# zaphB/freecad.optics_design_workbench

Measured on AMD Instinct MI355X. Metric: Monte-Carlo rays/sec (whole node), lensesAndMirrors.FCStd, higher is better.
Workload: dtype f64; 1 GPU; benchmark/lensesAndMirrors.FCStd, 1e+08 Monte-Carlo rays per step per GPU (BASELINE configs[2]), Gaussian point source sigma=1e-2, Philox4x32-10 seed 0x0D15EA5E; record_hit_rows=True, histogram=1024x1024 u64, parallelism=ray-index sharding x1, one RCCL reduce

## Files before the change

### freecad/optics_design_workbench_amd/csrc/odw_capi.hip

```cpp
#include <hip/hip_runtime.h>
#include <hipcub/hipcub.hpp>

#include <algorithm>
#include <array>
#include <cmath>
#include <cstdio>
#include <cstdlib>
#include <cstring>
#include <condition_variable>
#include <functional>
#include <mutex>
#include <new>
#include <thread>
#include <string>
#include <utility>
#include <vector>

#include "odw_kernels.hip"
#include "odw_grid.hip"
#include "odw_mesh.hip"

using namespace odw;

namespace {
// ... 2150 lines not shown
  }
  return ODW_OK;
}

namespace {
void batch_unselect(odw_ctx* ctx) {
  if (ctx->batch_selected < 0 && !ctx->archive_selected) return;
  ctx->archive_selected = false;
  ctx->hits = ctx->own_hits;
  ctx->hit_count = ctx->own_hit_count;
  ctx->hit_capacity = ctx->own_capacity;
  ctx->hit_slots = ctx->own_slots;
  ctx->hit_ray_begin = ctx->own_ray_begin;
  ctx->hit_ray_end = ctx->own_ray_end;
  ctx->own_hits = DevBuf();
  ctx->own_hit_count = DevBuf();
  ctx->batch_selected = -1;
  ctx->ph_valid = false;
}

bool same_structure(const odw_ctx& a, const odw_ctx& b, std::string& why) {
  if (a.P.scene.n_prims != b.P.scene.n_prims || a.P.scene.n_groups != b.P.scene.n_groups) { why = "primitive or group count"; return false; }
  for (size_t i = 0; i < a.h_prim_i32.size(); ++i) {
    const int32_t mask = (i % 4 == 2) ? ~(int32_t)ODW_FLAG_ISOLATED : ~0;
    if ((a.h_prim_i32[i] & mask) != (b.h_prim_i32[i] & mask)) { why = "primitive kinds, groups, flags or trimming lists"; return false; }
  }
  if (a.h_cond != b.h_cond) { why = "trimming conditions"; return false; }
  if (a.h_group_i32 != b.h_group_i32) { why = "optical types / recording switches / grating kinds"; return false; }
  if (a.h_seq != b.h_seq || a.P.scene.seq_enabled != b.P.scene.seq_enabled || a.P.scene.seq_len != b.P.scene.seq_len ||
      a.P.scene.ignore_mask != b.P.scene.ignore_mask) { why = "tracing sequence / ignored groups"; return false; }
  if (a.lean != b.lean) { why = "gratings or absorbing media in some scenes only"; return false; }
  return true;
}
}

int odw_upload_scene_batch(odw_ctx* ctx, const odw_scene_desc* scenes, int32_t n_scenes) {
  if (!ctx || !scenes || n_scenes < 1) return fail(ctx, ODW_ERR_INVALID, "odw_upload_scene_batch: bad argument");
  if (!ctx->have_limits) return fail(ctx, ODW_ERR_NO_SCENE, "odw_upload_scene_batch before odw_set_limits (the boxes carry the tolerance)");
  HIPCHK(ctx, hipSetDevice(ctx->device));
  ctx->batch_n = 0;
  ctx->batch_traced = 0;
  ctx->batch_rows_ok = false;
  ctx->phb_valid = ctx->phb_projected = false;
  int rc = odw_upload_scene(ctx, &scenes[0]);
  if (rc) return rc;
  if ((rc = build_bvh(ctx))) return rc;
  if (ctx->P.scene.n_nodes || ctx->P.grid.nx > 0)
    return fail(ctx, ODW_ERR_UNSUPPORTED, "odw_upload_scene_batch: batches are traced by the flat kernels (analytic scenes of up to 64 primitives)");
  const bool compiled = ctx->compile_mode != ODW_COMPILE_OFF && spec_ineligible(ctx).empty();
  const std::string text0 = compiled ? spec_text(ctx) : std::string();
  const size_t n = (size_t)ctx->P.scene.n_prims;
  const size_t o_hdr = 16 * n, o_gf = o_hdr + 8 * n, o_gd = o_gf + ODW_MAX_GROUPS * 4, stride = o_gd + ODW_MAX_GROUPS * 3;
  std::vector<double> blocks(stride * (size_t)n_scenes, 0.0);
  for (int k = 0; k < n_scenes; ++k) {
    odw_ctx tmp;
    std::memset(&tmp.P, 0, sizeof tmp.P);
    if ((rc = scene_host_tables(&tmp, &scenes[k]))) { ctx->err = tmp.err; g_error = tmp.err; return rc; }
    std::string why;
    if (!same_structure(*ctx, tmp, why))
      return fail(ctx, ODW_ERR_UNSUPPORTED, "odw_upload_scene_batch: scene " + std::to_string(k) + " differs from scene 0 in structure (" + why + ")");
    tmp.P.lim = ctx->P.lim;
    tmp.have_limits = true;
    std::vector<Box> boxes;
    std::vector<char> dead;
    compute_boxes(&tmp, boxes, dead);
    if (compiled && spec_text(&tmp) != text0)
      return fail(ctx, ODW_ERR_UNSUPPORTED, "odw_upload_scene_batch: scene " + std::to_string(k) + " differs from scene 0 in the structure a "
                                            "compiled kernel is built from (which frame entries are 0 / +1 / -1, shared boxes)");
    double* b = blocks.data() + stride * (size_t)k;
    std::memcpy(b, tmp.h_prim_f64.data(), 16 * n * sizeof(double));
    std::memcpy(b + o_hdr, tmp.h_prim_hdr.data(), 8 * n * sizeof(double));
    for (size_t p = 0; p < n; ++p) {
      int32_t w[4];
      std::memcpy(w, b + o_hdr + 8 * p + 6, sizeof w);
      w[2] &= ~ODW_FLAG_ISOLATED;
      std::memcpy(b + o_hdr + 8 * p + 6, w, sizeof w);
    }
    std::memcpy(b + o_gf, tmp.h_group_f64.data(), ODW_MAX_GROUPS * 4 * sizeof(double));
    std::memcpy(b + o_gd, tmp.h_group_gdir.data(), ODW_MAX_GROUPS * 3 * sizeof(double));
  }
  if ((rc = upload(ctx, ctx->batch_values, blocks.data(), blocks.size() * sizeof(double)))) return rc;
  std::vector<int32_t> pi = ctx->h_prim_i32;
  for (size_t p = 0; p < n; ++p) pi[4 * p + 2] &= ~ODW_FLAG_ISOLATED;
  if (n && (rc = upload(ctx, ctx->prim_i32, pi.data(), pi.size() * sizeof(int32_t)))) return rc;
  if ((rc = upload_done(ctx))) return rc;
  ctx->h_prim_i32 = pi;
  ctx->batch_n = n_scenes;
  ctx->batch_prims = n;
  ctx->batch_stride = stride;
  ctx->batch_spec_text = text0;
  return ODW_OK;
}

namespace {
uint64_t batch_slots(odw_ctx* ctx, uint64_t rows_per_scene) {
  uint64_t slots = rows_per_scene;
  if (rows_per_scene >= kHitBlockMinRows)
    slots += hit_block_room(rows_per_scene, std::min<uint64_t>((uint64_t)ctx->n_cu * 8 * 4, std::max<uint64_t>(64, rows_per_scene / 256)), kHitBlock);
  return slots;
}
}

int odw_batch_reserve(odw_ctx* ctx, int32_t n_scenes, uint64_t rays_per_scene, uint64_t rows_per_scene) {
  if (!ctx || n_scenes < 1 || rays_per_scene == 0) return fail(ctx, ODW_ERR_INVALID, "odw_batch_reserve: bad argument");
  HIPCHK(ctx, hipSetDevice(ctx->device));
  const uint64_t S = (uint64_t)n_scenes, slots = batch_slots(ctx, rows_per_scene);
  if (slots > 0x7FFFFFFFull) return fail(ctx, ODW_ERR_CAPACITY, "odw_batch_reserve: more than 2^31 rows per scene");
  HIPCHK(ctx, hipStreamSynchronize(ctx->stream));
  int rc = ODW_OK;
  if (rows_per_scene) {
    rc = ensure(ctx, ctx->batch_hits, S * slots * sizeof(odw_hit));
    if (!rc) rc = ensure(ctx, ctx->batch_hit_count, S * 4 * sizeof(uint64_t));
  }
  if (!rc) rc = phb_reserve(ctx, (int)S, rays_per_scene, slots);
  if (!rc && rows_per_scene && rays_per_scene <= (1ull << 28))
    rc = ensure(ctx, ctx->phb_pts, S * slots * 3 * sizeof(double));
  if (!rc && S >= 3) rc = ensure(ctx, ctx->batch_rays_buf, (size_t)((rays_per_scene + 31) / 32 * 32 * 6 + 4) * sizeof(double));
  return rc;
}

int odw_trace_batch(odw_ctx* ctx, uint64_t first_ray, uint64_t rays_per_scene, uint64_t seed, uint32_t flags,
                    uint64_t rows_per_scene) {
  if (!ctx) return fail(ctx, ODW_ERR_INVALID, "odw_trace_batch: null ctx");
  if (ctx->batch_n < 1)
    return fail(ctx, ODW_ERR_NO_SCENE, "odw_trace_batch before odw_upload_scene_batch (odw_upload_scene and a new dist_tol discard an uploaded batch)");
  if (ctx->bvh_dirty || (size_t)ctx->P.scene.n_prims != ctx->batch_prims)
    return fail(ctx, ODW_ERR_NO_SCENE, "odw_trace_batch: the scene changed after odw_upload_scene_batch");
  if (ctx->emitter_active) return fail(ctx, ODW_ERR_UNSUPPORTED, "odw_trace_batch: point sources only");
  if (rays_per_scene == 0) return ODW_OK;
  HIPCHK(ctx, hipSetDevice(ctx->device));
  batch_unselect(ctx);
  ctx->batch_rows_ok = false;
  const uint64_t S = (uint64_t)ctx->batch_n;
  if (flags & ODW_TRACE_RECORD_HITS) {
    if (rows_per_scene == 0) return fail(ctx, ODW_ERR_CAPACITY, "odw_trace_batch: ODW_TRACE_RECORD_HITS with rows_per_scene = 0");
    const uint64_t slots = batch_slots(ctx, rows_per_scene);
// ... 515 lines not shown
```

### freecad/optics_design_workbench_amd/csrc/odw_device.h

```cpp
#pragma once
#ifndef __HIPCC_RTC__
#include <hip/hip_runtime.h>
#include <stdint.h>
#else
typedef signed char int8_t;
typedef unsigned char uint8_t;
typedef signed int int32_t;
typedef unsigned int uint32_t;
typedef signed long int64_t;
typedef unsigned long uint64_t;
typedef unsigned long uintptr_t;
#endif

#ifdef __HIPCC_RTC__
#include "odw_trace.h"
#else
#include "../../../include/odw_trace.h"
#endif

#ifndef INFINITY
#define INFINITY (__builtin_inff())
#endif

namespace odw {

#define ODW_TAG_UNUSED 0xFFFFFFFFFFFFFFFFull
#define ODW_CNT_LDS 8
#define ODW_SOLID_SHIFT 16
#define ODW_FLAG_ISOLATED 0x4

__host__ __device__ __forceinline__ constexpr int cond_operand(int cw) { return cw & 0x3fffffff; }
__host__ __device__ __forceinline__ constexpr bool cond_opens(int cw) { return (cw & 0x40000000) != 0; }

struct d3 {
  double x, y, z;
};
__device__ __forceinline__ d3 mk(double x, double y, double z) { return d3{x, y, z}; }
__device__ __forceinline__ d3 operator+(d3 a, d3 b) { return mk(a.x + b.x, a.y + b.y, a.z + b.z); }
__device__ __forceinline__ d3 operator-(d3 a, d3 b) { return mk(a.x - b.x, a.y - b.y, a.z - b.z); }
__device__ __forceinline__ d3 operator*(d3 a, double s) { return mk(a.x * s, a.y * s, a.z * s); }
__device__ __forceinline__ double dot(d3 a, d3 b) { return a.x * b.x + a.y * b.y + a.z * b.z; }
__device__ __forceinline__ d3 cross(d3 a, d3 b) {
  return mk(a.y * b.z - a.z * b.y, a.z * b.x - a.x * b.z, a.x * b.y - a.y * b.x);
}
__device__ __forceinline__ double comp(d3 a, int i) { return i == 0 ? a.x : (i == 1 ? a.y : a.z); }

struct DeviceScene {
  const double* prim_f64;
  const double* prim_hdr;
  const int32_t* prim_i32;
  const int32_t* cond_i32;
  const double* group_f64;
  const int32_t* group_i32;
  const double* group_gdir;
  const uint64_t* seq_mask;
  const float* bvh_nodes;
  const int32_t* bvh_prims;
  const float* bvh_leaf;
  const uint32_t* bvh_wide;
  double wide_lo[3], wide_hi[3];
  const double* tri_nrm;
  int32_t n_prims, n_groups, n_nodes;
  int32_t seq_enabled, seq_len;
  uint64_t ignore_mask, all_mask;
};

struct DeviceGrid {
  const double* bounds;
  const uint32_t* cells;
  const void* items;
  int32_t nx, ny, nz, n_items;
  int32_t spheres;
  int32_t in_lds;
  uint32_t lds_bytes;
};

struct DeviceSource {
  double m[12];
  double focal_length, wavelength, power;
  const double* phi_tab;
  const double* t_tab;
  const int32_t* t_guide;
  const int32_t* phi_guide;
  int32_t n_phi_knots, n_t_knots, n_t_rows, n_guide, n_phi_guide;
  int32_t finite_focal;
};

struct DeviceSurfaceSampler {
  const double* phi_tab;
  const double* t_tab;
  const int32_t* t_guide;
  int32_t n_phi_knots, n_t_knots, n_t_rows, n_guide;
  int32_t axis, n_family;
  double lo, inv_step;
  double mu;
  int32_t next;
  int32_t n_atoms;
  const double* atom_mass;
// ... 79 lines not shown
```

### freecad/optics_design_workbench_amd/csrc/odw_grid.hip

```cpp
#include "odw_device.h"

namespace odw {

#ifndef ODW_GRID_STEP_MIN
#define ODW_GRID_STEP_MIN 24
#endif
#ifndef ODW_GRID_REFILL_MIN
#define ODW_GRID_REFILL_MIN 1
#endif
#define ODW_GRID_THREADS 1024
#define ODW_GRID_WAVES (ODW_GRID_THREADS / 64)
#define ODW_GRID_WAVE_WORDS 32
#define ODW_GRID_RING 64
#define ODW_GRID_RING_DOUBLES (ODW_GRID_RING * 7)

#ifdef ODW_GRID_STATS
#define ODW_GSTAT(k, mask_)                                                                           \
  do {                                                                                                \
    const unsigned long long m_ = (mask_);                                                            \
    if (m_ && (int)__lane_id() == __ffsll(m_) - 1) { wave_cnt[8 + 2 * (k)] += 1u; wave_cnt[9 + 2 * (k)] += (uint32_t)__popcll(m_); } \
  } while (0)
#define ODW_GTIME(k) do { const uint64_t t_ = __builtin_readcyclecounter(); phase_t[(k)] += t_ - t_mark; t_mark = t_; } while (0)
#else
#define ODW_GSTAT(k, mask_) do {} while (0)
#define ODW_GTIME(k) do {} while (0)
#endif

__device__ __forceinline__ double fmin_raw(double a, double b) {
  double r;
  asm("v_min_f64 %0, %1, %2" : "=v"(r) : "v"(a), "v"(b));
  return r;
}

__device__ __forceinline__ int grid_slab(const double* b, int n, double v) {
  int lo = 0, hi = n;
  while (hi - lo > 1) {
    const int mid = (lo + hi) >> 1;
    if (v >= b[mid]) lo = mid; else hi = mid;
  }
  return lo;
}

#define ODW_GCOUNT(k) atomicAdd(&wave_cnt[(k)], 1u)

template <bool SPHERES, bool IN_LDS>
__global__ __launch_bounds__(ODW_GRID_THREADS) void odw_grid_kernel(const TraceParams P) {
  extern __shared__ double grid_lds[];
  const DeviceScene& sc = P.scene;
  const DeviceLimits& lim = P.lim;
  const DeviceGrid& GD = P.grid;
  const int nx = GD.nx, ny = GD.ny, nz = GD.nz;
  const int nb = nx + ny + nz + 3;
  const int ncell = nx * ny * nz;
  uint32_t* lds32 = reinterpret_cast<uint32_t*>(grid_lds);
  const int word_off = 2 * nb;
  const int ring_off = (word_off + ODW_GRID_WAVES * ODW_GRID_WAVE_WORDS + 1) / 2;
  const int cell_off = 2 * (ring_off + ODW_GRID_WAVES * ODW_GRID_RING_DOUBLES);
  const int item_off = ((cell_off + (IN_LDS ? ncell : 0) + 3) & ~3) / 2;
  for (int k = threadIdx.x; k < nb; k += ODW_GRID_THREADS) grid_lds[k] = GD.bounds[k];
  for (int k = threadIdx.x; k < ODW_GRID_WAVES * ODW_GRID_WAVE_WORDS; k += ODW_GRID_THREADS)
    lds32[word_off + k] = (k % ODW_GRID_WAVE_WORDS) == 30 ? P.out.hit_block : 0u;
  if (IN_LDS) {
    for (int k = threadIdx.x; k < ncell; k += ODW_GRID_THREADS) lds32[cell_off + k] = GD.cells[k];
    const int n_words = SPHERES ? GD.n_items * 6 : (GD.n_items + 1) / 2;
    const double* src = reinterpret_cast<const double*>(GD.items);
    for (int k = threadIdx.x; k < n_words; k += ODW_GRID_THREADS) grid_lds[item_off + k] = src[k];
  }
  __syncthreads();
  const double* bx = grid_lds;
  const int by_off = nx + 1, bz_off = nx + ny + 2;
  const int wave = threadIdx.x >> 6;
  uint32_t* wave_cnt = lds32 + word_off + wave * ODW_GRID_WAVE_WORDS;
  volatile uint32_t* hit_state = wave_cnt + 28;
  double* ring = grid_lds + ring_off + wave * ODW_GRID_RING_DOUBLES;

  SceneView sv;
  sv.prim_f64 = as_const(sc.prim_f64);
  sv.prim_hdr = as_const(sc.prim_hdr);
  sv.prim_i32 = as_const(sc.prim_i32);
  sv.cond_i32 = as_const(sc.cond_i32);
  __shared__ double group_f64[64 * 4];
  __shared__ int32_t group_i32[64 * 4];
  __shared__ double group_gdir[64 * 3];
  {
    cf64 gf = as_const(sc.group_f64);
// ... 400 lines not shown
```

### freecad/optics_design_workbench_amd/csrc/odw_kernels.hip

```cpp
#include "odw_device.h"

namespace odw {

#define ODW_CONST __attribute__((address_space(4)))
typedef const double ODW_CONST* cf64;
typedef const int32_t ODW_CONST* ci32;
typedef const uint64_t ODW_CONST* cu64;
template <class T>
__device__ __forceinline__ const T ODW_CONST* as_const(const T* p) {
  return (const T ODW_CONST*)(uintptr_t)p;
}
template <class T>
__device__ __forceinline__ const T* opaque(const T* p) {
  asm volatile("" : "+s"(p));
  return p;
}
typedef const DeviceSource ODW_CONST* csource;
typedef const DeviceDetector ODW_CONST* cdetector;

__device__ __forceinline__ double frcp(double x) {
  double r = __builtin_amdgcn_rcp(x);
  r = fma(fma(-x, r, 1.0), r, r);
  r = fma(fma(-x, r, 1.0), r, r);
  return r;
// ... 318 lines not shown
    }
    if (!held) return;
  }
  if (cand_any) { q.any.t = t; q.any.prim = p; q.any.face = face; }
  if (cand_oth) { q.oth.t = t; q.oth.prim = p; q.oth.face = face; }
}

template <bool PARAB, class SPEC, int C, int END>
__device__ __forceinline__ bool trim_all(const SceneView& sv, const Query& q, d3 gp) {
  if constexpr (C >= END) {
    return true;
  } else {
    constexpr int cw = SPEC::cond(C);
    constexpr int qp = cond_operand(cw);
    cf64 pf = sv.prim_f64 + (size_t)qp * 16;
    const double sd = prim_sdist<PARAB>(SPEC::type(qp), pf + 12, xf_point_nz<SPEC::xf(qp)>(pf, gp));
    if (cw < 0) { if (sd > q.tol) return false; }
    else { if (sd < -q.tol) return false; }
    return trim_all<PARAB, SPEC, C + 1, END>(sv, q, gp);
  }
}
template <class SPEC>
__host__ __device__ constexpr int clause_end(int c, int end) {
  int e = c + 1;
  while (e < end && !cond_opens(SPEC::cond(e))) ++e;
  return e;
}
template <bool PARAB, class SPEC, int C, int END>
__device__ __forceinline__ bool trim_ok(const SceneView& sv, const Query& q, d3 gp) {
  constexpr int E = clause_end<SPEC>(C, END);
  if constexpr (E >= END) {
    return trim_all<PARAB, SPEC, C, END>(sv, q, gp);
  } else {
    if (trim_all<PARAB, SPEC, C, E>(sv, q, gp)) return true;
    return trim_ok<PARAB, SPEC, E, END>(sv, q, gp);
  }
}
template <bool PARAB, class SPEC, int PI>
__device__ __forceinline__ void consider_spec(const SceneView& sv, Query& q, double t, int face) {
  if (!(t > q.tol && t < q.tmax)) return;
  const int key = (PI << 8) | face;
#define ODW_BETTER(B) ((bool)((int)(t < (B).t) | ((int)(t == (B).t) & (int)(key < (B).face))))
  const bool cand_any = ODW_BETTER(q.any);
  bool cand_oth = false;
  if (q.in_medium) cand_oth = (SPEC::group(PI) != q.medium) && (q.medium >= 0) && ODW_BETTER(q.oth);
#undef ODW_BETTER
  if (!cand_any && !cand_oth) return;
  if constexpr (SPEC::cond_cnt(PI) > 0) {
    if (!trim_ok<PARAB, SPEC, SPEC::cond_off(PI), SPEC::cond_off(PI) + SPEC::cond_cnt(PI)>(sv, q, q.start + q.dn * t)) return;
#if ODW_DOUBLE == 5
    if (!trim_ok<PARAB, SPEC, SPEC::cond_off(PI), SPEC::cond_off(PI) + SPEC::cond_cnt(PI)>(sv, q, q.start + q.dn * opq(t))) return;
#endif
  }
  if (cand_any) { q.any.t = t; q.any.face = key; q.cut = fmin(q.tmax, t + 2.0 * q.tol); }
  if (cand_oth) { q.oth.t = t; q.oth.face = key; }
}

struct Cands {
  double t0, t1, t2, t3;
  int f0, f1, f2, f3;
};
__device__ __forceinline__ void cand_push(Cands& c, int& n, double t, int f) {
  if (n == 0) { c.t0 = t; c.f0 = f; }
  else if (n == 1) { c.t1 = t; c.f1 = f; }
  else if (n == 2) { c.t2 = t; c.f2 = f; }
  else { c.t3 = t; c.f3 = f; }
  ++n;
}
__device__ __forceinline__ void cand_min2(Cands& c, double t, int f) {
  const bool lt0 = t < c.t0 || (t == c.t0 && f < c.f0);
  const bool lt1 = t < c.t1 || (t == c.t1 && f < c.f1);
  c.t1 = lt0 ? c.t0 : (lt1 ? t : c.t1);
  c.f1 = lt0 ? c.f0 : (lt1 ? f : c.f1);
  c.t0 = lt0 ? t : c.t0;
  c.f0 = lt0 ? f : c.f0;
}

#ifndef ODW_TORUS_PLAIN
#define ODW_TORUS_PLAIN 96
#endif
template <bool PARAB = true, class SPEC = NoSpec, int PI = 0>
__device__ __forceinline__ void intersect_prim(const SceneView& sv, Query& q, int p, int type, int group,
                                               int flags, int cond_word) {
  cf64 pf = sv.prim_f64 + (size_t)p * 16;
  const int cond_off = cond_word & 0xffffff, cond_cnt = (cond_word >> 24) & 0xff;
  const int fmask = (flags >> ODW_FACEMASK_SHIFT) & 0xff;
  cf64 par = pf + 12;
  const double tol = q.tol;
  Cands c;
  c.t0 = c.t1 = c.t2 = c.t3 = INFINITY;
  c.f0 = c.f1 = c.f2 = c.f3 = 0;
  if (type == ODW_PRIM_SPHERE) {
    if (fmask & 1) {
      const d3 oc = q.start - mk(par[1], par[2], par[3]);
      double t0, t1;
      if (quad_roots_unit(dot(oc, q.dn), dot(oc, oc) - par[0] * par[0], t0, t1) == 2) {
        c.t0 = t0;
        c.t1 = t1;
      }
#if ODW_DOUBLE == 2
      {
        const d3 oc2 = mk(opq(oc.x), oc.y, oc.z);
        double u0 = INFINITY, u1 = INFINITY;
        if (quad_roots_unit(dot(oc2, q.dn), dot(oc2, oc2) - par[0] * par[0], u0, u1) == 2) { c.t0 = u0 == c.t0 ? c.t0 : u0; c.t1 = u1 == c.t1 ? c.t1 : u1; }
      }
#endif
    }
  } else {
  d3 o, d;
  if constexpr (SPEC::enabled) {
    o = xf_point_nz<SPEC::xf(PI)>(pf, q.start);
    d = xf_vec_nz<SPEC::xf(PI)>(pf, q.dn);
  } else {
    o = xf_point(pf, q.start);
    d = xf_vec(pf, q.dn);
  }
  if (type == ODW_PRIM_BOX) {
    const double ix = frcp(d.x), iy = frcp(d.y), iz = frcp(d.z);
    const double ax = -o.x * ix, ay = -o.y * iy, az = -o.z * iz;
    const double bx = fma(par[0], ix, ax), by = fma(par[1], iy, ay), bz = fma(par[2], iz, az);
    const bool px = d.x > 0, py = d.y > 0, pz = d.z > 0;
    const double nx_ = fmin(ax, bx), ny_ = fmin(ay, by), nz_ = fmin(az, bz);
    const double fx_ = fmax(ax, bx), fy_ = fmax(ay, by), fz_ = fmax(az, bz);
    if (cond_cnt) {
#define ODW_BOX_FACE2(T, FACE, P1, D1, S1, P2, D2, S2, TA, FA, TB, FB)                          \
      {                                                                                         \
        const double t_ = (T);                                                                  \
        const double u_ = fma(t_, D1, P1), v_ = fma(t_, D2, P2);                                \
        const bool ok_ = ((fmask >> (FACE)) & 1) && t_ > tol && u_ >= -tol && u_ <= (S1) + tol && \
                         v_ >= -tol && v_ <= (S2) + tol;                                        \
        const bool a_ = ok_ && t_ < TA;                                                         \
        const bool b_ = ok_ && !a_ && t_ < TB;                                                  \
        TB = a_ ? TA : (b_ ? t_ : TB);                                                          \
        FB = a_ ? FA : (b_ ? (FACE) : FB);                                                      \
        TA = a_ ? t_ : TA;                                                                      \
        FA = a_ ? (FACE) : FA;                                                                  \
      }
      ODW_BOX_FACE2(nx_, px ? 0 : 1, o.y, d.y, par[1], o.z, d.z, par[2], c.t0, c.f0, c.t2, c.f2);
      ODW_BOX_FACE2(ny_, py ? 2 : 3, o.z, d.z, par[2], o.x, d.x, par[0], c.t0, c.f0, c.t2, c.f2);
      ODW_BOX_FACE2(nz_, pz ? 4 : 5, o.x, d.x, par[0], o.y, d.y, par[1], c.t0, c.f0, c.t2, c.f2);
      ODW_BOX_FACE2(fx_, px ? 1 : 0, o.y, d.y, par[1], o.z, d.z, par[2], c.t1, c.f1, c.t3, c.f3);
      ODW_BOX_FACE2(fy_, py ? 3 : 2, o.z, d.z, par[2], o.x, d.x, par[0], c.t1, c.f1, c.t3, c.f3);
      ODW_BOX_FACE2(fz_, pz ? 5 : 4, o.x, d.x, par[0], o.y, d.y, par[1], c.t1, c.f1, c.t3, c.f3);
#undef ODW_BOX_FACE2
    } else {
    double bt = INFINITY;
    int bf = 0;
#define ODW_BOX_OK(A, B, C, D, E, F) (bool)((int)(A) & (int)(B) & (int)(C) & (int)(D) & (int)(E) & (int)(F))
#define ODW_BOX_FACE(T, FACE, P1, D1, S1, P2, D2, S2)                                         \
    {                                                                                         \
      const double t_ = (T);                                                                  \
      const double u_ = fma(t_, D1, P1), v_ = fma(t_, D2, P2);                                \
      const bool ok_ = ODW_BOX_OK(((fmask >> (FACE)) & 1) != 0, t_ > tol, u_ >= -tol, u_ <= (S1) + tol, \
                                  v_ >= -tol, v_ <= (S2) + tol);                              \
      if (ok_ && (t_ < bt || (t_ == bt && (FACE) < bf))) { bt = t_; bf = (FACE); }            \
    }
    ODW_BOX_FACE(nx_, px ? 0 : 1, o.y, d.y, par[1], o.z, d.z, par[2]);
    ODW_BOX_FACE(ny_, py ? 2 : 3, o.z, d.z, par[2], o.x, d.x, par[0]);
    ODW_BOX_FACE(nz_, pz ? 4 : 5, o.x, d.x, par[0], o.y, d.y, par[1]);
    c.t0 = bt;
    c.f0 = bf;
    const double t_in = fmax(fmax(nx_, ny_), nz_);
    const double t_out = fmin(fmin(fx_, fy_), fz_);
    if (!(bt < INFINITY) || !(t_in < t_out)) {
      bt = INFINITY;
      bf = 0;
      ODW_BOX_FACE(fx_, px ? 1 : 0, o.y, d.y, par[1], o.z, d.z, par[2]);
      ODW_BOX_FACE(fy_, py ? 3 : 2, o.z, d.z, par[2], o.x, d.x, par[0]);
      ODW_BOX_FACE(fz_, pz ? 5 : 4, o.x, d.x, par[0], o.y, d.y, par[1]);
      c.t1 = bt;
      c.f1 = bf;
    }
#undef ODW_BOX_FACE
#undef ODW_BOX_OK
    }
  } else if (type == ODW_PRIM_CYLINDER || type == ODW_PRIM_CONE || (PARAB && type == ODW_PRIM_PARABOLOID)) {
    const bool parab = PARAB && type == ODW_PRIM_PARABOLOID;
    const double R1 = parab ? 0.0 : par[0];
    const double R2 = (type == ODW_PRIM_CYLINDER) ? par[0] : (parab ? par[2] : par[1]);
    const double H = (type == ODW_PRIM_CONE) ? par[2] : par[1];
    const double k = (type == ODW_PRIM_CONE) ? (R2 - R1) / H : 0.0;
    const double f2 = parab ? 2.0 * par[0] : 0.0;
    constexpr bool side_skip = SPEC::enabled || !PARAB;
    bool side = (fmask & 1) != 0;
    double invz = 0.0;
    if ((fmask & 6) || (side_skip && type == ODW_PRIM_CYLINDER && side)) invz = frcp(d.z);
    if (side_skip && type == ODW_PRIM_CYLINDER && side) {
      const double tl = (-tol - o.z) * invz, th = (H + tol - o.z) * invz;
      const double xl = fma(tl, d.x, o.x), yl = fma(tl, d.y, o.y), xh = fma(th, d.x, o.x), yh = fma(th, d.y, o.y);
      const double lim = R1 * R1 * (1.0 - 1e-9);
      side = !(fma(xl, xl, yl * yl) < lim && fma(xh, xh, yh * yh) < lim);
    }
    if (side) {
      const double rz = R1 + k * o.z;
      double t0 = INFINITY, t1 = INFINITY;
      const int nr = quad_roots(d.x * d.x + d.y * d.y - k * k * d.z * d.z,
                                o.x * d.x + o.y * d.y - k * rz * d.z - f2 * d.z,
                                o.x * o.x + o.y * o.y - rz * rz - 2.0 * f2 * o.z, t0, t1);
      const double z0 = o.z + t0 * d.z, z1 = o.z + t1 * d.z;
      c.t0 = (bool)((int)(nr >= 1) & (int)(z0 >= -tol) & (int)(z0 <= H + tol) & (int)((R1 + k * z0) >= -tol)) ? t0 : c.t0;
      c.t1 = (bool)((int)(nr == 2) & (int)(z1 >= -tol) & (int)(z1 <= H + tol) & (int)((R1 + k * z1) >= -tol)) ? t1 : c.t1;
    }
    if (fmask & 6) {
      const double ta = (0.0 - o.z) * invz, tb = (H - o.z) * invz;
      const double xa = o.x + ta * d.x, ya = o.y + ta * d.y;
      const double xb = o.x + tb * d.x, yb = o.y + tb * d.y;
      { const bool w_ = (bool)((int)((fmask & 2) != 0) & (int)(R1 > 0) & (int)(xa * xa + ya * ya <= (R1 + tol) * (R1 + tol))); c.t2 = w_ ? ta : c.t2; c.f2 = w_ ? 1 : c.f2; }
      { const bool w_ = (bool)((int)((fmask & 4) != 0) & (int)(R2 > 0) & (int)(xb * xb + yb * yb <= (R2 + tol) * (R2 + tol))); c.t3 = w_ ? tb : c.t3; c.f3 = w_ ? 2 : c.f3; }
    }
  } else {
    if (!(fmask & 1)) return;
    const double R1 = par[0], R2 = par[1];
    const double t0 = -dot(o, d);
    const d3 cc = o + d * t0;
    const double bound = (R1 + R2) * 1.0000001 + 1e-9;
    const double h2 = bound * bound - dot(cc, cc);
// ... 138 lines not shown
}

__device__ __forceinline__ d3 tri_normal(cf64 pf, const double* __restrict__ vn, d3 gp) {
  const d3 ng = mk(pf[9], pf[10], pf[11]);
  if (!vn) return ng;
  const d3 e1 = mk(pf[3], pf[4], pf[5]), e2 = mk(pf[6], pf[7], pf[8]);
  const d3 tv = gp - mk(pf[0], pf[1], pf[2]);
  const d3 nn = cross(e1, e2);
  const double inv = frcp(dot(nn, nn));
  const double u = dot(cross(tv, e2), nn) * inv, v = dot(cross(e1, tv), nn) * inv;
  const double w = 1.0 - u - v;
  const d3 n = mk(w * vn[0] + u * vn[3] + v * vn[6], w * vn[1] + u * vn[4] + v * vn[7],
                  w * vn[2] + u * vn[5] + v * vn[8]);
  const double l2 = dot(n, n);
  return l2 > 0 ? n * frsqrt(l2) : ng;
}

template <bool PARAB = true>
__device__ __forceinline__ d3 face_normal(int type, cf64 par, int face, d3 lp) {
  if (type == ODW_PRIM_BOX) {
    const double s = (face & 1) ? 1.0 : -1.0;
    const int a = face >> 1;
    return mk(a == 0 ? s : 0.0, a == 1 ? s : 0.0, a == 2 ? s : 0.0);
  }
  if (type == ODW_PRIM_SPHERE) return lp * frsqrt(dot(lp, lp));
  if (type == ODW_PRIM_CYLINDER || type == ODW_PRIM_CONE || (PARAB && type == ODW_PRIM_PARABOLOID)) {
    if (face == 1) return mk(0, 0, -1);
    if (face == 2) return mk(0, 0, 1);
    double k = 0;
    if (type == ODW_PRIM_CONE) k = (par[1] - par[0]) / par[2];
    const d3 g = mk(lp.x, lp.y, (PARAB && type == ODW_PRIM_PARABOLOID) ? -2.0 * par[0] : -k * (par[0] + k * lp.z));
    return g * frsqrt(dot(g, g));
  }
  const double f = 1.0 - par[0] * frsqrt(lp.x * lp.x + lp.y * lp.y);
  const d3 g = mk(lp.x * f, lp.y * f, lp.z);
  return g * frsqrt(dot(g, g));
}

#ifndef ODW_BVH_STACK
#define ODW_BVH_STACK 32
#endif
template <class P>
__device__ __forceinline__ bool ray_box(P bx, d3 oi, d3 inv, double tmax) {
  double t0 = fma(bx[0], inv.x, -oi.x), t1 = fma(bx[3], inv.x, -oi.x);
  double lo = fmin(t0, t1), hi = fmax(t0, t1);
  t0 = fma(bx[1], inv.y, -oi.y); t1 = fma(bx[4], inv.y, -oi.y);
  lo = fmax(lo, fmin(t0, t1)); hi = fmin(hi, fmax(t0, t1));
  t0 = fma(bx[2], inv.z, -oi.z); t1 = fma(bx[5], inv.z, -oi.z);
  lo = fmax(lo, fmin(t0, t1)); hi = fmin(hi, fmax(t0, t1));
  return hi >= fmax(lo, 0.0) && lo < tmax;
}

template <class SPEC, int PI>
__device__ __forceinline__ void spec_prim(const SceneView& sv, Query& q, d3 oi, d3 inv, int skip_solid, int only_solid,
                                          uint64_t mask, bool* boxhit) {
  constexpr int flags = SPEC::flags(PI);
  if constexpr (!SPEC::dead(PI) && (SPEC::seq() || ((SPEC::umask() >> SPEC::group(PI)) & 1) != 0)) {
    if ((!SPEC::seq() || ((mask >> SPEC::group(PI)) & 1)) && (flags >> ODW_SOLID_SHIFT) != skip_solid &&
        (!SPEC::isolated() || only_solid < 0 || (flags >> ODW_SOLID_SHIFT) == only_solid)) {
      bool in_box;
      if constexpr (SPEC::box_of(PI) != PI) {
        in_box = boxhit[SPEC::box_of(PI)];
      } else {
        const double cut = q.cut;
        in_box = ray_box(sv.prim_hdr + 8 * PI, oi, inv, cut);
#if ODW_DOUBLE == 1
        in_box = in_box & ray_box(sv.prim_hdr + 8 * PI, mk(opq(oi.x), oi.y, oi.z), inv, cut);
#endif
      }
      boxhit[PI] = in_box;
      if (in_box)
        intersect_prim<SPEC::parab(), SPEC, PI>(sv, q, PI, SPEC::type(PI), SPEC::group(PI), flags, SPEC::cond_word(PI));
#if ODW_DOUBLE == 3 || ODW_DOUBLE == 4 || ODW_DOUBLE == 12
      if (in_box && SPEC::type(PI) == (ODW_DOUBLE == 3 ? ODW_PRIM_CYLINDER : (ODW_DOUBLE == 4 ? ODW_PRIM_BOX : ODW_PRIM_SPHERE))) {
        Query q2 = q;
        q2.start.x = opq(q.start.x);
        intersect_prim<SPEC::parab(), SPEC, PI>(sv, q2, PI, SPEC::type(PI), SPEC::group(PI), flags, SPEC::cond_word(PI));
        q.any = q2.any; q.oth = q2.oth;
      }
#endif
    } else if constexpr (SPEC::box_of(PI) == PI) {
      boxhit[PI] = SPEC::box_shared(PI) ? ray_box(sv.prim_hdr + 8 * PI, oi, inv, q.cut) : false;
    }
  }
}
template <class T, T... I> struct IndexList {};
template <class SPEC, int... PI>
__device__ __forceinline__ void spec_prims(const SceneView& sv, Query& q, d3 oi, d3 inv, int skip_solid, int only_solid,
                                           uint64_t mask, IndexList<int, PI...>) {
  bool boxhit[sizeof...(PI)] = {};
  (spec_prim<SPEC, PI>(sv, q, oi, inv, skip_solid, only_solid, mask, boxhit), ...);
}

template <bool BVH, class SPEC = NoSpec>
__device__ __forceinline__ int nearest(const DeviceScene& sc, const SceneView& sv,
                                       const DeviceLimits& lim, d3 start, d3 dn, int medium,
                                       uint64_t mask, double& t_hit, int& face,
                                       int* __restrict__ stack, int skip_solid, int only_solid = -1) {
  Query q;
  q.start = start; q.dn = dn; q.tol = lim.dist_tol; q.tmax = lim.max_ray_length + lim.dist_tol;
  q.medium = medium;
  q.in_medium = __ballot(medium >= 0) != 0ull;
  q.cut = q.tmax;
  q.any.t = INFINITY; q.any.prim = 0x7fffffff; q.any.face = 0x7fffffff;
  q.oth = q.any;
#if ODW_DOUBLE == 9
  d3 inv = mk(frcp1(dn.x), frcp1(dn.y), frcp1(dn.z));
  d3 oi = mk(start.x * inv.x, start.y * inv.y, start.z * inv.z);
  {
    const d3 dn2 = mk(opq(dn.x), opq(dn.y), opq(dn.z));
    const d3 inv2 = mk(frcp1(dn2.x), frcp1(dn2.y), frcp1(dn2.z));
    const d3 oi2 = mk(start.x * inv2.x, start.y * inv2.y, start.z * inv2.z);
    inv = inv2.x == inv.x ? inv : inv2;
    oi = oi2.y == oi.y ? oi : oi2;
  }
#else
  const d3 inv = mk(frcp1(dn.x), frcp1(dn.y), frcp1(dn.z));
  const d3 oi = mk(start.x * inv.x, start.y * inv.y, start.z * inv.z);
#endif
  if constexpr (SPEC::enabled) {
    spec_prims<SPEC>(sv, q, oi, inv, skip_solid, only_solid, mask, __make_integer_seq<IndexList, int, SPEC::N>{});
  } else if (!BVH) {
    const bool per_lane_mask = sc.seq_enabled != 0;
    const uint64_t umask = sc.all_mask & ~sc.ignore_mask;
    for (int p = 0; p < sc.n_prims; ++p) {
      cf64 hdr = sv.prim_hdr + 8 * p;
      ci32 hi = (ci32)(hdr + 6);
      const int type = hi[0], g = hi[1], flags = hi[2], cond_word = hi[3];
      if (per_lane_mask) {
        if (!((mask >> g) & 1)) continue;
      } else {
        if (!((umask >> g) & 1)) continue;
      }
      if ((flags >> ODW_SOLID_SHIFT) == skip_solid) continue;
      if (only_solid >= 0 && (flags >> ODW_SOLID_SHIFT) != only_solid) continue;
      const double cut = fmin(q.tmax, q.any.t + 2.0 * q.tol);
      if (!ray_box(hdr, oi, inv, cut)) continue;
      intersect_prim<false>(sv, q, p, type, g, flags, cond_word);
    }
  } else {
    typedef const float ODW_CONST* cf32;
    typedef float vf4 __attribute__((ext_vector_type(4)));
    typedef int vi4 __attribute__((ext_vector_type(4)));
    cf32 nodes = (cf32)(uintptr_t)sc.bvh_nodes;
    ci32 bvh_prims = as_const(sc.bvh_prims);
    const float ofx = (float)start.x, ofy = (float)start.y, ofz = (float)start.z;
    const float ivx = (float)inv.x, ivy = (float)inv.y, ivz = (float)inv.z;
    int sp = 0;
    int cur = 0;
    int pend = -1;
    for (;;) {
      for (;;) {
        const unsigned long long looking = __ballot(cur >= 0 && pend == -1);
        if (!(cur >= 0 && (pend == -1 || looking != 0ull))) break;
        cf32 nd = nodes + (size_t)cur * 16;
        const vf4 a0 = *reinterpret_cast<const vf4 ODW_CONST*>(nd);
        const vf4 a1 = *reinterpret_cast<const vf4 ODW_CONST*>(nd + 4);
        const vf4 a2 = *reinterpret_cast<const vf4 ODW_CONST*>(nd + 8);
        const vi4 lk = *reinterpret_cast<const vi4 ODW_CONST*>(nd + 12);
        const float cutf = (float)fmin(q.tmax, q.any.t + 2.0 * q.tol) * 1.00001f + 1e-3f;
        float tn0, tf0, tn1, tf1;
        {
          const float x0 = (a0.x - ofx) * ivx, x1 = (a0.w - ofx) * ivx;
          const float y0 = (a0.y - ofy) * ivy, y1 = (a1.x - ofy) * ivy;
          const float z0 = (a0.z - ofz) * ivz, z1 = (a1.y - ofz) * ivz;
          tn0 = fmaxf(fmaxf(fminf(x0, x1), fminf(y0, y1)), fminf(z0, z1));
          tf0 = fminf(fminf(fmaxf(x0, x1), fmaxf(y0, y1)), fmaxf(z0, z1));
        }
        {
          const float x0 = (a1.z - ofx) * ivx, x1 = (a2.y - ofx) * ivx;
          const float y0 = (a1.w - ofy) * ivy, y1 = (a2.z - ofy) * ivy;
          const float z0 = (a2.x - ofz) * ivz, z1 = (a2.w - ofz) * ivz;
          tn1 = fmaxf(fmaxf(fminf(x0, x1), fminf(y0, y1)), fminf(z0, z1));
          tf1 = fminf(fminf(fmaxf(x0, x1), fmaxf(y0, y1)), fmaxf(z0, z1));
// ... 375 lines not shown
    ++seq;
  } else {
    const d3 gd = mk(group_gdir[3 * g], group_gdir[3 * g + 1], group_gdir[3 * g + 2]);
    const double lpm = group_f64[4 * g + 3];
    const int order = group_i32[4 * g + 3];
    if (group_i32[4 * g + 2] == 0) {
      if (entering) {
        const double nn = (medium >= 0) ? group_f64[4 * medium] : 1.0;
        dir = line_grating(dir, nn, nn, n, P.wavelength, order, lpm, gd, false);
        ++seq;
      }
    } else if (entering) {
      if (medium >= 0) {
        atomicAdd(P.out.counters + ODW_CNT_GRATING_IN_MEDIUM, 1ull);
        cnt[ODW_CNT_DIED * 256] += 1u;
        alive = false;
      }
      medium = g;
      dir = line_grating(dir, 1.0, group_f64[4 * g], n, P.wavelength, order, lpm, gd, true);
    } else {
      const double n1 = (medium >= 0) ? group_f64[4 * medium] : 1.0;
      bool tir;
      dir = snells_law(dir, n1, 1.0, n, tir);
      if (!tir) { medium = -1; ++seq; }
    }
  }
}

template <bool STOCH, bool LEAN, class SPEC, int PI>
__device__ __forceinline__ void spec_hit(const TraceParams& P, const SceneView& sv, cf64 group_f64, ci32 group_i32,
                                         cf64 group_gdir, int face, uint64_t ray, int nint, uint32_t* cnt,
                                         uint32_t* hit_state, uint32_t* win, d3 point, d3& dir, double& power, int& medium, int& seq,
                                         int& skip, int& only, bool& alive) {
  constexpr int flags = SPEC::flags(PI), g = SPEC::group(PI);
  cf64 pf = sv.prim_f64 + (size_t)PI * 16;
  d3 n = face_normal<SPEC::parab()>(SPEC::type(PI), pf + 12, face, xf_point_nz<SPEC::xf(PI)>(pf, point));
  if constexpr ((flags & ODW_FLAG_FLIP_NORMAL) != 0) n = n * -1.0;
  n = xf_vec_t_nz<SPEC::xf(PI)>(pf, n);
#if ODW_DOUBLE == 6
  {
    d3 n2 = face_normal<SPEC::parab()>(SPEC::type(PI), pf + 12, face, xf_point_nz<SPEC::xf(PI)>(pf, mk(opq(point.x), point.y, point.z)));
    if constexpr ((flags & ODW_FLAG_FLIP_NORMAL) != 0) n2 = n2 * -1.0;
    n2 = xf_vec_t_nz<SPEC::xf(PI)>(pf, n2);
    n = n2.x == n.x ? n : n2;
  }
#endif
  const bool entering = dot(dir, n) < 0;
  if (entering) n = n * -1.0;
  interact<false, STOCH, LEAN>(P, group_f64, group_i32, group_gdir, g, SPEC::gtype(g), SPEC::record(g), n, entering, ray,
                               nint, cnt, hit_state, win, point, dir, power, medium, seq, alive);
  const double out = entering ? -dot(dir, n) : dot(dir, n);
  if constexpr ((flags & ODW_FLAG_CONVEX) != 0) skip = out > 0 ? (flags >> ODW_SOLID_SHIFT) : -1;
  else skip = -1;
  if constexpr ((flags & ODW_FLAG_ISOLATED) != 0) only = out < 0 ? (flags >> ODW_SOLID_SHIFT) : -1;
  else only = -1;
}
template <bool STOCH, bool LEAN, class SPEC, int... PI>
__device__ __forceinline__ void spec_hits(const TraceParams& P, const SceneView& sv, cf64 group_f64, ci32 group_i32,
                                          cf64 group_gdir, int prim, int face, uint64_t ray, int nint, uint32_t* cnt,
                                          uint32_t* hit_state, uint32_t* win, d3 point, d3& dir, double& power, int& medium, int& seq,
                                          int& skip, int& only, bool& alive, IndexList<int, PI...>) {
  (void)((prim == PI ? (spec_hit<STOCH, LEAN, SPEC, PI>(P, sv, group_f64, group_i32, group_gdir, face, ray, nint, cnt, hit_state, win,
                                                  point, dir, power, medium, seq, skip, only, alive), true)
                     : false) || ...);
}

__device__ __forceinline__ void close_hit_block(const TraceParams& P, volatile uint32_t* hit_state, uint32_t next_scene) {
  if (!P.out.hit_block) {
    if (P.batch.n_scenes && __lane_id() == 0) hit_state[3] = next_scene;
    return;
  }
  odw_hit* hits = P.out.hits;
  unsigned long long* hit_count = P.out.hit_count;
  if (P.batch.n_scenes) {
    const uint32_t cur = __builtin_amdgcn_readfirstlane(hit_state[3]);
    hits += (size_t)cur * P.out.hit_capacity;
    hit_count += 4 * cur;
  }
  const uint32_t hit_used = hit_state[2];
  const uint64_t hit_base = ((uint64_t)hit_state[1] << 32) | hit_state[0];
  if (hit_used < P.out.hit_block) {
    const uint32_t left = P.out.hit_block - hit_used;
    for (uint32_t k = __lane_id(); k < left; k += 64)
      if (hit_base + hit_used + k < P.out.hit_capacity) hits[hit_base + hit_used + k].tag = ODW_TAG_UNUSED;
    const uint64_t at = hit_base + hit_used;
    const uint64_t in_buf = at < P.out.hit_capacity ? (P.out.hit_capacity - at < left ? P.out.hit_capacity - at : left) : 0;
    if (__lane_id() == 0 && in_buf) atomicAdd(hit_count + 1, (unsigned long long)in_buf);
  }
  if (__lane_id() == 0) {
    hit_state[0] = 0u; hit_state[1] = 0u; hit_state[2] = P.out.hit_block; hit_state[3] = next_scene;
  }
}

template <bool ON> struct HitBlockState {
  __device__ static __forceinline__ uint32_t* lds() {
    __shared__ uint32_t state[4 * 4 + 4 + ODW_HIST_WIN * ODW_HIST_WIN];
    return state;
  }
};
template <> struct HitBlockState<false> {
  __device__ static __forceinline__ uint32_t* lds() { return nullptr; }
};

#ifndef ODW_CHUNK
#define ODW_CHUNK 2048ull
#endif
#ifndef ODW_REFILL_MIN
#define ODW_REFILL_MIN 16
// ... 439 lines not shown
```

### freecad/optics_design_workbench_amd/csrc/odw_spec.hip

```cpp
#include <dlfcn.h>
#include <hip/hiprtc.h>
#include <sys/stat.h>
#include <unistd.h>

#include <atomic>
#include <chrono>
#include <map>
#include <memory>
#include <mutex>
#include <thread>

#if !defined(__HIP_DEVICE_COMPILE__)
__asm__(
    ".pushsection .rodata\n"
    ".global odw_src_kernels\nodw_src_kernels:\n.incbin \"odw_kernels.hip\"\n.byte 0\n"
    ".global odw_src_device\nodw_src_device:\n.incbin \"odw_device.h\"\n.byte 0\n"
    ".global odw_src_trace\nodw_src_trace:\n.incbin \"../../../include/odw_trace.h\"\n.byte 0\n"
    ".popsection\n");
#endif
extern "C" const char odw_src_kernels[], odw_src_device[], odw_src_trace[];

namespace {

int spec_max_prims() {
// ... 75 lines not shown
    flags[p] = ctx->h_prim_i32[4 * p + 2] & ~ODW_FLAG_ISOLATED;
    condw[p] = ctx->h_prim_i32[4 * p + 3];
    const int facemask = (flags[p] >> ODW_FACEMASK_SHIFT) & 0xff;
    dead[p] = facemask == 0;
    const double* m = &ctx->h_prim_f64[16 * (size_t)p];
    unsigned long long w = 0;
    for (int i = 0; i < 12; ++i) {
      if (m[i] != 0.0) w |= 1ull << i;
      if (i % 4 != 3 && m[i] == 1.0) w |= 1ull << (12 + i);
      if (i % 4 != 3 && m[i] == -1.0) w |= 1ull << (24 + i);
    }
    xf[p] = w;
  }
  std::vector<int> box_of(n), box_shared(n, 0);
  {
    std::vector<std::vector<std::vector<int>>> inside(n);
    for (int p = 0; p < n; ++p) {
      const int off = condw[p] & 0xffffff, cnt = (condw[p] >> 24) & 0xff;
      const int end = std::min(off + cnt, (int)ctx->h_cond.size());
      inside[p].push_back({p});
      for (int c = off; c < end; ++c) {
        if (c != off && cond_opens(ctx->h_cond[c])) inside[p].push_back({p});
        if (ctx->h_cond[c] < 0) inside[p].back().push_back(cond_operand(ctx->h_cond[c]));
      }
      for (std::vector<int>& set : inside[p]) {
        std::sort(set.begin(), set.end());
        set.erase(std::unique(set.begin(), set.end()), set.end());
      }
      std::sort(inside[p].begin(), inside[p].end());
    }
    for (int p = 0; p < n; ++p) {
      box_of[p] = p;
      for (int q = 0; q < p; ++q)
        if (!dead[q] && !dead[p] && group[q] == group[p] && inside[q] == inside[p]) { box_of[p] = q; box_shared[q] = 1; break; }
    }
  }
  std::vector<int> gtype(std::max(1, ng)), grec(std::max(1, ng));
  for (int g = 0; g < ng; ++g) { gtype[g] = ctx->h_group_i32[4 * g]; grec[g] = ctx->h_group_i32[4 * g + 1]; }
  auto fi = [](int v) { return std::to_string(v); };
  auto fu = [](unsigned long long v) { char b[32]; snprintf(b, sizeof b, "0x%llxull", v); return std::string(b); };
  std::string s;
  s += "struct Spec {\n  static constexpr bool enabled = true;\n";
  s += "  static constexpr int N = " + std::to_string(n) + ";\n";
  s += table("int", "type", n, type.data(), fi) + table("int", "group", n, group.data(), fi) +
       table("int", "flags", n, flags.data(), fi) + table("int", "cond_word", n, condw.data(), fi) +
       table("bool", "dead", n, dead.data(), fi) + table("int", "box_of", n, box_of.data(), fi) +
       table("bool", "box_shared", n, box_shared.data(), fi) +
       table("int", "cond", (int)ctx->h_cond.size(), ctx->h_cond.data(), fi) +
       table("unsigned long long", "xf", n, xf.data(), fu) + table("int", "gtype", ng, gtype.data(), fi) +
       table("bool", "record", ng, grec.data(), fi);
  bool parab = false;
  for (int p = 0; p < n; ++p) parab |= type[p] == ODW_PRIM_PARABOLOID;
  s += std::string("  static constexpr bool parab() { return ") + (parab ? "true" : "false") + "; }\n";
  s += "  static constexpr bool isolated() { return false; }\n";
  s += "  static constexpr int cond_off(int i) { return cond_word(i) & 0xffffff; }\n"
       "  static constexpr int cond_cnt(int i) { return (cond_word(i) >> 24) & 0xff; }\n";
  s += "  static constexpr unsigned long long umask() { return " + fu(ctx->P.scene.all_mask & ~ctx->P.scene.ignore_mask) + "; }\n";
  s += std::string("  static constexpr bool seq() { return ") + (ctx->P.scene.seq_enabled ? "true" : "false") + "; }\n";
  s += "};\n";
  s += std::string("#define ODW_SPEC_LEAN ") + (ctx->lean ? "true" : "false") + "\n";
  s += std::string("#define ODW_SPEC_STOCH ") + (ctx->n_samplers > 0 ? "true" : "false") + "\n";
  return s;
}

uint64_t fnv1a(const std::string& s, uint64_t h = 1469598103934665603ull) {
  for (unsigned char c : s) { h ^= c; h *= 1099511628211ull; }
  return h;
}

std::string cache_dir() {
  const char* e = getenv("ODW_KERNEL_CACHE");
  if (e) return *e ? e : "";
  const char* x = getenv("XDG_CACHE_HOME");
  if (x && *x) return std::string(x) + "/odw_trace";
  const char* h = getenv("HOME");
  return h && *h ? std::string(h) + "/.cache/odw_trace" : "";
}

void mkdirs(const std::string& path) {
  for (size_t i = 1; i <= path.size(); ++i)
    if (i == path.size() || path[i] == '/') (void)mkdir(path.substr(0, i).c_str(), 0755);
}

bool spec_compile(const std::string& text, const std::string& arch, std::vector<char>& code, std::string& err) {
  Hiprtc& rtc = hiprtc();
  if (!rtc.error.empty()) { err = rtc.error; return false; }
  const char* headers[] = {odw_src_kernels, odw_src_device, odw_src_trace, text.c_str()};
  const char* names[] = {"odw_kernels.hip", "odw_device.h", "odw_trace.h", "odw_spec.h"};
  hiprtcProgram prog = nullptr;
  if (rtc.create(&prog, "#include \"odw_kernels.hip\"\n", "odw_spec_kernel.hip", 4, headers, names) != HIPRTC_SUCCESS) {
    err = "hiprtcCreateProgram failed";
    return false;
  }
  const std::string a = "--offload-arch=" + arch;
  std::vector<const char*> opts = {a.c_str(), "-std=c++17", "-O3", "-ffp-contract=on", "-DODW_SPEC_HEADER=\"odw_spec.h\""};
  std::vector<std::string> extra;
  if (const char* e = getenv("ODW_SPEC_OPTS")) {
    std::string w;
    for (const char* c = e;; ++c) {
      if (*c == ' ' || *c == 0) { if (!w.empty()) extra.push_back(w); w.clear(); if (!*c) break; }
      else w += *c;
    }
  }
  for (const std::string& x : extra) opts.push_back(x.c_str());
  const hiprtcResult r = rtc.compile(prog, (int)opts.size(), opts.data());
  if (r != HIPRTC_SUCCESS) {
    size_t ls = 0;
// ... 210 lines not shown
```

Measured before the change: 9.549 billion rays/s.

## Enable isolated-solid wave-uniform culling in compiled kernels and use raw f64 min/max

The compiled spec kernel now treats the isolated flag as live. When every lane in a wave is confined to the same isolated solid, primitives of other solids are skipped and box tests and reciprocal setup are bypassed. The batch upload keeps the isolated flag only where it holds for all scenes, and the per-hit 'only' solid is read from device prim flags at runtime. Separately, fmin/fmax in box slab tests are replaced with raw v_min/v_max_f64 inline asm, which drops IEEE NaN-handling overhead. This adds a readfirstlane/ballot and a global load per hit, and changes NaN semantics in the slab test.

```diff
diff --git a/freecad/optics_design_workbench_amd/csrc/odw_capi.hip b/freecad/optics_design_workbench_amd/csrc/odw_capi.hip
--- a/freecad/optics_design_workbench_amd/csrc/odw_capi.hip
+++ b/freecad/optics_design_workbench_amd/csrc/odw_capi.hip
@@ -2226,6 +2226,7 @@
   const size_t n = (size_t)ctx->P.scene.n_prims;
   const size_t o_hdr = 16 * n, o_gf = o_hdr + 8 * n, o_gd = o_gf + ODW_MAX_GROUPS * 4, stride = o_gd + ODW_MAX_GROUPS * 3;
   std::vector<double> blocks(stride * (size_t)n_scenes, 0.0);
+  std::vector<int32_t> isolated(n, ODW_FLAG_ISOLATED);
   for (int k = 0; k < n_scenes; ++k) {
     odw_ctx tmp;
     std::memset(&tmp.P, 0, sizeof tmp.P);
@@ -2244,18 +2245,21 @@
     double* b = blocks.data() + stride * (size_t)k;
     std::memcpy(b, tmp.h_prim_f64.data(), 16 * n * sizeof(double));
     std::memcpy(b + o_hdr, tmp.h_prim_hdr.data(), 8 * n * sizeof(double));
-    for (size_t p = 0; p < n; ++p) {
-      int32_t w[4];
-      std::memcpy(w, b + o_hdr + 8 * p + 6, sizeof w);
-      w[2] &= ~ODW_FLAG_ISOLATED;
-      std::memcpy(b + o_hdr + 8 * p + 6, w, sizeof w);
-    }
+    for (size_t p = 0; p < n; ++p) isolated[p] &= tmp.h_prim_i32[4 * p + 2];
     std::memcpy(b + o_gf, tmp.h_group_f64.data(), ODW_MAX_GROUPS * 4 * sizeof(double));
     std::memcpy(b + o_gd, tmp.h_group_gdir.data(), ODW_MAX_GROUPS * 3 * sizeof(double));
   }
+  for (int k = 0; k < n_scenes; ++k)
+    for (size_t p = 0; p < n; ++p) {
+      double* h = blocks.data() + stride * (size_t)k + o_hdr + 8 * p;
+      int32_t w[4];
+      std::memcpy(w, h + 6, sizeof w);
+      w[2] = (w[2] & ~ODW_FLAG_ISOLATED) | isolated[p];
+      std::memcpy(h + 6, w, sizeof w);
+    }
   if ((rc = upload(ctx, ctx->batch_values, blocks.data(), blocks.size() * sizeof(double)))) return rc;
   std::vector<int32_t> pi = ctx->h_prim_i32;
-  for (size_t p = 0; p < n; ++p) pi[4 * p + 2] &= ~ODW_FLAG_ISOLATED;
+  for (size_t p = 0; p < n; ++p) pi[4 * p + 2] = (pi[4 * p + 2] & ~ODW_FLAG_ISOLATED) | isolated[p];
   if (n && (rc = upload(ctx, ctx->prim_i32, pi.data(), pi.size() * sizeof(int32_t)))) return rc;
   if ((rc = upload_done(ctx))) return rc;
   ctx->h_prim_i32 = pi;
diff --git a/freecad/optics_design_workbench_amd/csrc/odw_device.h b/freecad/optics_design_workbench_amd/csrc/odw_device.h
--- a/freecad/optics_design_workbench_amd/csrc/odw_device.h
+++ b/freecad/optics_design_workbench_amd/csrc/odw_device.h
@@ -44,6 +44,17 @@
   return mk(a.y * b.z - a.z * b.y, a.z * b.x - a.x * b.z, a.x * b.y - a.y * b.x);
 }
 __device__ __forceinline__ double comp(d3 a, int i) { return i == 0 ? a.x : (i == 1 ? a.y : a.z); }
+
+__device__ __forceinline__ double fmin_raw(double a, double b) {
+  double r;
+  asm("v_min_f64 %0, %1, %2" : "=v"(r) : "v"(a), "v"(b));
+  return r;
+}
+__device__ __forceinline__ double fmax_raw(double a, double b) {
+  double r;
+  asm("v_max_f64 %0, %1, %2" : "=v"(r) : "v"(a), "v"(b));
+  return r;
+}
 
 struct DeviceScene {
   const double* prim_f64;
diff --git a/freecad/optics_design_workbench_amd/csrc/odw_grid.hip b/freecad/optics_design_workbench_amd/csrc/odw_grid.hip
--- a/freecad/optics_design_workbench_amd/csrc/odw_grid.hip
+++ b/freecad/optics_design_workbench_amd/csrc/odw_grid.hip
@@ -26,11 +26,6 @@
 #define ODW_GTIME(k) do {} while (0)
 #endif
 
-__device__ __forceinline__ double fmin_raw(double a, double b) {
-  double r;
-  asm("v_min_f64 %0, %1, %2" : "=v"(r) : "v"(a), "v"(b));
-  return r;
-}
 
 __device__ __forceinline__ int grid_slab(const double* b, int n, double v) {
   int lo = 0, hi = n;
diff --git a/freecad/optics_design_workbench_amd/csrc/odw_kernels.hip b/freecad/optics_design_workbench_amd/csrc/odw_kernels.hip
--- a/freecad/optics_design_workbench_amd/csrc/odw_kernels.hip
+++ b/freecad/optics_design_workbench_amd/csrc/odw_kernels.hip
@@ -394,7 +394,7 @@
     if (!trim_ok<PARAB, SPEC, SPEC::cond_off(PI), SPEC::cond_off(PI) + SPEC::cond_cnt(PI)>(sv, q, q.start + q.dn * opq(t))) return;
 #endif
   }
-  if (cand_any) { q.any.t = t; q.any.face = key; q.cut = fmin(q.tmax, t + 2.0 * q.tol); }
+  if (cand_any) { q.any.t = t; q.any.face = key; q.cut = fmin_raw(q.tmax, t + 2.0 * q.tol); }
   if (cand_oth) { q.oth.t = t; q.oth.face = key; }
 }
 
@@ -462,8 +462,8 @@
     const double ax = -o.x * ix, ay = -o.y * iy, az = -o.z * iz;
     const double bx = fma(par[0], ix, ax), by = fma(par[1], iy, ay), bz = fma(par[2], iz, az);
     const bool px = d.x > 0, py = d.y > 0, pz = d.z > 0;
-    const double nx_ = fmin(ax, bx), ny_ = fmin(ay, by), nz_ = fmin(az, bz);
-    const double fx_ = fmax(ax, bx), fy_ = fmax(ay, by), fz_ = fmax(az, bz);
+    const double nx_ = fmin_raw(ax, bx), ny_ = fmin_raw(ay, by), nz_ = fmin_raw(az, bz);
+    const double fx_ = fmax_raw(ax, bx), fy_ = fmax_raw(ay, by), fz_ = fmax_raw(az, bz);
     if (cond_cnt) {
 #define ODW_BOX_FACE2(T, FACE, P1, D1, S1, P2, D2, S2, TA, FA, TB, FB)                          \
       {                                                                                         \
@@ -502,8 +502,8 @@
     ODW_BOX_FACE(nz_, pz ? 4 : 5, o.x, d.x, par[0], o.y, d.y, par[1]);
     c.t0 = bt;
     c.f0 = bf;
-    const double t_in = fmax(fmax(nx_, ny_), nz_);
-    const double t_out = fmin(fmin(fx_, fy_), fz_);
+    const double t_in = fmax_raw(fmax_raw(nx_, ny_), nz_);
+    const double t_out = fmin_raw(fmin_raw(fx_, fy_), fz_);
     if (!(bt < INFINITY) || !(t_in < t_out)) {
       bt = INFINITY;
       bf = 0;
@@ -748,14 +748,18 @@
 }
 
 template <class SPEC, int PI>
-__device__ __forceinline__ void spec_prim(const SceneView& sv, Query& q, d3 oi, d3 inv, int skip_solid, int only_solid,
-                                          uint64_t mask, bool* boxhit) {
+__device__ __forceinline__ void spec_prim(const SceneView& sv, Query& q, const d3& oi, const d3& inv, int skip_solid,
+                                          int wave_solid, uint64_t mask, bool* boxhit) {
   constexpr int flags = SPEC::flags(PI);
   if constexpr (!SPEC::dead(PI) && (SPEC::seq() || ((SPEC::umask() >> SPEC::group(PI)) & 1) != 0)) {
-    if ((!SPEC::seq() || ((mask >> SPEC::group(PI)) & 1)) && (flags >> ODW_SOLID_SHIFT) != skip_solid &&
-        (!SPEC::isolated() || only_solid < 0 || (flags >> ODW_SOLID_SHIFT) == only_solid)) {
+    const bool ruled = SPEC::isolated() && wave_solid >= 0;
+    if (ruled && (flags >> ODW_SOLID_SHIFT) != wave_solid) {
+      if constexpr (SPEC::box_of(PI) == PI) boxhit[PI] = false;
+    } else if ((!SPEC::seq() || ((mask >> SPEC::group(PI)) & 1)) && (flags >> ODW_SOLID_SHIFT) != skip_solid) {
       bool in_box;
-      if constexpr (SPEC::box_of(PI) != PI) {
+      if (ruled) {
+        in_box = true;
+      } else if constexpr (SPEC::box_of(PI) != PI) {
         in_box = boxhit[SPEC::box_of(PI)];
       } else {
         const double cut = q.cut;
@@ -776,16 +780,16 @@
       }
 #endif
     } else if constexpr (SPEC::box_of(PI) == PI) {
-      boxhit[PI] = SPEC::box_shared(PI) ? ray_box(sv.prim_hdr + 8 * PI, oi, inv, q.cut) : false;
+      boxhit[PI] = (SPEC::box_shared(PI) && !ruled) ? ray_box(sv.prim_hdr + 8 * PI, oi, inv, q.cut) : false;
     }
   }
 }
 template <class T, T... I> struct IndexList {};
 template <class SPEC, int... PI>
-__device__ __forceinline__ void spec_prims(const SceneView& sv, Query& q, d3 oi, d3 inv, int skip_solid, int only_solid,
-                                           uint64_t mask, IndexList<int, PI...>) {
+__device__ __forceinline__ void spec_prims(const SceneView& sv, Query& q, const d3& oi, const d3& inv, int skip_solid,
+                                           int wave_solid, uint64_t mask, IndexList<int, PI...>) {
   bool boxhit[sizeof...(PI)] = {};
-  (spec_prim<SPEC, PI>(sv, q, oi, inv, skip_solid, only_solid, mask, boxhit), ...);
+  (spec_prim<SPEC, PI>(sv, q, oi, inv, skip_solid, wave_solid, mask, boxhit), ...);
 }
 
 template <bool BVH, class SPEC = NoSpec>
@@ -800,22 +804,25 @@
   q.cut = q.tmax;
   q.any.t = INFINITY; q.any.prim = 0x7fffffff; q.any.face = 0x7fffffff;
   q.oth = q.any;
+  int wave_solid = -1;
+  if constexpr (SPEC::enabled && SPEC::isolated()) {
+    const int u = __builtin_amdgcn_readfirstlane(only_solid);
+    if (u >= 0 && __ballot(only_solid != u) == 0ull) wave_solid = u;
+  }
+  d3 inv, oi;
+  if (wave_solid < 0) {
+    inv = mk(frcp1(dn.x), frcp1(dn.y), frcp1(dn.z));
+    oi = mk(start.x * inv.x, start.y * inv.y, start.z * inv.z);
 #if ODW_DOUBLE == 9
-  d3 inv = mk(frcp1(dn.x), frcp1(dn.y), frcp1(dn.z));
-  d3 oi = mk(start.x * inv.x, start.y * inv.y, start.z * inv.z);
-  {
     const d3 dn2 = mk(opq(dn.x), opq(dn.y), opq(dn.z));
     const d3 inv2 = mk(frcp1(dn2.x), frcp1(dn2.y), frcp1(dn2.z));
     const d3 oi2 = mk(start.x * inv2.x, start.y * inv2.y, start.z * inv2.z);
     inv = inv2.x == inv.x ? inv : inv2;
     oi = oi2.y == oi.y ? oi : oi2;
-  }
-#else
-  const d3 inv = mk(frcp1(dn.x), frcp1(dn.y), frcp1(dn.z));
-  const d3 oi = mk(start.x * inv.x, start.y * inv.y, start.z * inv.z);
-#endif
+#endif
+  }
   if constexpr (SPEC::enabled) {
-    spec_prims<SPEC>(sv, q, oi, inv, skip_solid, only_solid, mask, __make_integer_seq<IndexList, int, SPEC::N>{});
+    spec_prims<SPEC>(sv, q, oi, inv, skip_solid, wave_solid, mask, __make_integer_seq<IndexList, int, SPEC::N>{});
   } else if (!BVH) {
     const bool per_lane_mask = sc.seq_enabled != 0;
     const uint64_t umask = sc.all_mask & ~sc.ignore_mask;
@@ -1297,8 +1304,7 @@
   const double out = entering ? -dot(dir, n) : dot(dir, n);
   if constexpr ((flags & ODW_FLAG_CONVEX) != 0) skip = out > 0 ? (flags >> ODW_SOLID_SHIFT) : -1;
   else skip = -1;
-  if constexpr ((flags & ODW_FLAG_ISOLATED) != 0) only = out < 0 ? (flags >> ODW_SOLID_SHIFT) : -1;
-  else only = -1;
+  only = ((sv.prim_i32[4 * PI + 2] & ODW_FLAG_ISOLATED) != 0 && out < 0) ? (flags >> ODW_SOLID_SHIFT) : -1;
 }
 template <bool STOCH, bool LEAN, class SPEC, int... PI>
 __device__ __forceinline__ void spec_hits(const TraceParams& P, const SceneView& sv, cf64 group_f64, ci32 group_i32,
diff --git a/freecad/optics_design_workbench_amd/csrc/odw_spec.hip b/freecad/optics_design_workbench_amd/csrc/odw_spec.hip
--- a/freecad/optics_design_workbench_amd/csrc/odw_spec.hip
+++ b/freecad/optics_design_workbench_amd/csrc/odw_spec.hip
@@ -151,7 +151,7 @@
   bool parab = false;
   for (int p = 0; p < n; ++p) parab |= type[p] == ODW_PRIM_PARABOLOID;
   s += std::string("  static constexpr bool parab() { return ") + (parab ? "true" : "false") + "; }\n";
-  s += "  static constexpr bool isolated() { return false; }\n";
+  s += "  static constexpr bool isolated() { return true; }\n";
   s += "  static constexpr int cond_off(int i) { return cond_word(i) & 0xffffff; }\n"
        "  static constexpr int cond_cnt(int i) { return (cond_word(i) >> 24) & 0xff; }\n";
   s += "  static constexpr unsigned long long umask() { return " + fu(ctx->P.scene.all_mask & ~ctx->P.scene.ignore_mask) + "; }\n";
```

Measured after the change: 8.977 billion rays/s. 6.0% lower.
